# Farofeiro231/LiDAR_SLAM

Measured on AMD Instinct MI355X. Metric: scans/sec (RANSAC+UKF, 720-pt scans) at 1/2/4/8 MI355X + HBM GB/s vs peak, higher is better.
Workload: dtype f64; 1 GPU; C3: 4096 synthetic 720-pt scans per GPU, chunked 7x100+20; RANSAC (100 trials, 20 mm, mt19937 hypotheses) + landmark association + UKF predict/update (n=3, L=20); scans_per_gpu=4096, trials=100, landmarks=20, hyp=mt19937, parallelism=dp1 (scan shards, no collective)

## Files before the change

lidar_slam_amd/csrc/lslam_rng_pipe.h:

```cpp
#pragma once
#include "../../include/lidarslam.h"
#include "lslam_rng.h"

namespace lslam {

#ifndef RP_PRIO_TOP
#define RP_PRIO_TOP 3
#endif
__device__ __forceinline__ void set_prio_level(int lvl) {
    switch (lvl) {
        case 3: __builtin_amdgcn_s_setprio(3); break;
        case 2: __builtin_amdgcn_s_setprio(2); break;
        case 1: __builtin_amdgcn_s_setprio(1); break;
        default: __builtin_amdgcn_s_setprio(0); break;
    }
}

template <int LO, int HI>
__device__ __forceinline__ void mt_twist_group(const uint32_t *src, uint32_t *dst, uint32_t *pad, int lane) {
    uint32_t a[HI - LO], b[HI - LO], c[HI - LO];
#pragma unroll
    for (int k = LO; k < HI; k++) {
        const int i = 64 * k + lane;
        if (k < 9 || i < MT_N) {
            a[k - LO] = src[i];
            b[k - LO] = src[i + 1];
            const uint32_t *f = (i < MT_N - MT_M) ? src + i + MT_M : dst + i - (MT_N - MT_M);
            c[k - LO] = *f;
        }
    }
#pragma unroll
    for (int k = LO; k < HI; k++) {
        const int i = 64 * k + lane;
        if (k < 9 || i < MT_N) {
            const uint32_t v = mt_mix(a[k - LO], b[k - LO], c[k - LO]);
            dst[i] = v;
            if (k == 0 && pad) pad[lane] = v;
        }
    }
    wave_lds_sync();
}
__device__ __forceinline__ void mt_twist_oop(const uint32_t *src, uint32_t *dst, uint32_t *pad, int lane) {
    mt_twist_group<0, 3>(src, dst, pad, lane);
    mt_twist_group<3, 6>(src, dst, pad, lane);
    mt_twist_group<6, 9>(src, dst, pad, lane);
    mt_twist_group<9, 10>(src, dst, pad, lane);
}

constexpr uint32_t RT_KMAX = 127;
constexpr int RT_ROWS = 128;
constexpr int RT_ST = 7;
constexpr int RT_DWORDS = RT_ROWS * RT_ST;
__host__ __device__ inline uint32_t rt_word(uint32_t K, uint32_t v, uint32_t q) {
    uint32_t word = 0;
    for (uint32_t b = 0; b < 32; b++) {
        const uint32_t x = q * 32u + b;
        const uint32_t i = K - x % K;
        uint32_t m = i;
        m |= m >> 1; m |= m >> 2; m |= m >> 4; m |= m >> 8; m |= m >> 16;
        if ((v & m) > i) word |= 1u << b;
    }
    return word;
}

struct RngPipe;
__device__ __forceinline__ int rp_level(const RngPipe &rp, uint32_t done);

struct RngPipe {
    uint32_t *blk;
    int have;
    uint32_t *tbl;
    uint32_t tblK;
    uint32_t total_steps;
    uint32_t lvl_t1, lvl_t2;
    uint32_t done_steps;
    int prio;
#ifdef LSLAM_STAMPS
    uint64_t acc[8];
#endif
#ifdef LSLAM_WSTAMPS
    uint64_t wacc[8];
#endif
};

__device__ __forceinline__ void rp_set_schedule(RngPipe &rp) {
    rp.lvl_t1 = (rp.total_steps + 1u + 2u) / 3u;
    rp.lvl_t2 = (2u * (rp.total_steps + 1u) + 2u) / 3u;
}
__device__ __forceinline__ int rp_level(const RngPipe &rp, uint32_t done) {
    return RP_PRIO_TOP - (done >= rp.lvl_t1 ? 1 : 0) - (done >= rp.lvl_t2 ? 1 : 0);
}

__device__ __forceinline__ void rp_need_block(RngPipe &rp, int need, int lane) {
    if (rp.have < need) {
        mt_twist_oop(rp.blk + ((need - 1) & 1) * MT_N, rp.blk + (need & 1) * MT_N,
                     (need & 1) == 0 ? rp.blk + 2 * MT_N : nullptr, lane);
        rp.have = need;
    }
}

#if defined(LSLAM_STAMPS) && !defined(LSLAM_WSTAMPS)
#define RP_STAMP_DECL uint64_t _rp_prev = lslam_stamp();
#define RP_STAMP(k)                         \
    do {                                    \
        const uint64_t _t = lslam_stamp();  \
        rp.acc[k] += _t - _rp_prev;         \
        _rp_prev = _t;                      \
    } while (0)
#define RP_COUNT(k, n) (rp.acc[k] += (n))
#else
#define RP_STAMP_DECL
#define RP_STAMP(k) do {} while (0)
#define RP_COUNT(k, n) do {} while (0)
#endif

__device__ __forceinline__ uint32_t mbcnt_from(uint64_t m, uint32_t base) {
    return __builtin_amdgcn_mbcnt_hi((uint32_t)(m >> 32), __builtin_amdgcn_mbcnt_lo((uint32_t)m, base));
}

__device__ __forceinline__ uint32_t step_mask(uint32_t i) { return 0xffffffffu >> __clz((int)i); }

__device__ __forceinline__ uint32_t rt_temper_mask(uint32_t y, uint32_t mK) {
    y ^= (y >> 11);
    y = __builtin_amdgcn_bitop3_b32(y << 7, 0x9d2c5680u, y, 0x6a);
    y = __builtin_amdgcn_bitop3_b32(y << 15, 0xefc60000u, y, 0x6a);
    return (y ^ (y >> 18)) & mK;
}

__device__ __forceinline__ uint32_t fy_index(uint32_t d, uint32_t K) { return min(d, d + K) + 1u; }
__device__ __forceinline__ uint32_t fy_j(uint32_t w, uint32_t i) { return w & (0xffffffffu >> __clz((int)i)); }

__device__ __forceinline__ void store_accepted(uint8_t *J, uint32_t idx, uint32_t v, uint64_t R) {
    uint64_t saved;
    asm volatile(
        "s_andn1_saveexec_b64 %0, %1\n\t"
        "global_store_byte %2, %3, %4\n\t"
        "s_mov_b64 exec, %0"
        : "=&s"(saved)
        : "s"(R), "v"(idx), "v"(v), "s"(J)
        : "memory", "scc");
}
__device__ __forceinline__ void store_accepted(uint16_t *J, uint32_t idx, uint32_t v, uint64_t R) {
    uint64_t saved;
    asm volatile(
        "s_andn1_saveexec_b64 %0, %1\n\t"
        "global_store_short %2, %3, %4\n\t"
        "s_mov_b64 exec, %0"
        : "=&s"(saved)
        : "s"(R), "v"(idx * 2u), "v"(v), "s"(J)
        : "memory", "scc");
}

__device__ __forceinline__ uint32_t accepted_count(uint64_t R) {
    uint32_t n;
    asm("s_bcnt0_i32_b64 %0, %1" : "=s"(n) : "s"(R) : "scc");
    return n;
}

template <bool FAST, typename JT>
__device__ __forceinline__ void parse_chunk(RngPipe &rp, int &blkno, int &pos, JT *__restrict__ J, uint32_t N,
                                            uint32_t D, int lane) {
    const uint32_t K = N - 1;
    const uint32_t G = D * K;
    const float invK = 1.0f / (float)K;
    const uint32_t guess = ((uint32_t)lane * 46u) >> 6;
    uint32_t g = 0, sg = 0;
    int pre_pos = -1;
    uint32_t pre_raw = 0;
    RP_STAMP_DECL
    while (g < G) {
        RP_STAMP(3);
        if (pos >= MT_N) {
            blkno += 1;
            rp_need_block(rp, blkno, lane);
            asm volatile("" ::: "memory");
            pos -= MT_N;
            pre_pos = -1;
            const int lvl = rp_level(rp, rp.done_steps + g);
            if (lvl != rp.prio) {
                rp.prio = lvl;
                set_prio_level(lvl);
            }
            RP_STAMP(0);
        }
        const uint32_t *kb = rp.blk + (blkno & 1) * MT_N;
        const uint32_t rem = G - g;
        if (FAST) {
            rp_need_block(rp, blkno + 1, lane);
            asm volatile("" ::: "memory");
        }
        const int nrun = FAST ? min((MT_N - pos + 63) >> 6, (int)((rem - 1u) >> 6)) : 0;
        if (nrun > 0) {
            uint32_t raw = (pre_pos == pos) ? pre_raw : kb[pos + lane];
            uint32_t w = rt_temper_mask(raw, 0xffffffffu);
            for (int r = 0; r < nrun; r++) {
                const uint32_t nraw = kb[pos + 64 + lane];
                RP_STAMP(3);
                const uint32_t b1 = K - 1u - sg;
                const uint32_t base0 = b1 - (uint32_t)lane;
                uint32_t d = b1 - guess;
                uint32_t i = fy_index(d, K);
                uint32_t jv = fy_j(w, i);
                uint64_t R = ballot(jv > i), Rp;
                const uint32_t wn = rt_temper_mask(nraw, 0xffffffffu);
                int it = 1;
                do {
                    Rp = R;
                    d = mbcnt_from(Rp, base0);
                    i = fy_index(d, K);
                    jv = fy_j(w, i);
                    R = ballot(jv > i);
                    it++;
                } while (R != Rp);
                (void)it;
                RP_STAMP(2);
                RP_COUNT(5, 1);
                RP_COUNT(6, it);
                store_accepted(J, g + (b1 - d), jv, R);
                const uint32_t na = accepted_count(R);
                pos += 64;
                g += na;
                sg += na;
                if (sg >= K) sg -= K;
                raw = nraw;
                w = wn;
            }
            pre_pos = pos;
            pre_raw = raw;
            continue;
        }
        const uint32_t raw = (pre_pos == pos) ? pre_raw : kb[min(pos + lane, MT_N - 1)];
        pre_pos = -1;
        const uint32_t w = mt_temper(raw);
        RP_STAMP(3);
        const int nw = min(64, MT_N - pos);
        const uint64_t actm = ballot(lane < nw);
        uint32_t c = guess, jv = 0;
        uint64_t B = 0;
        for (int it = 0;; it++) {
            const uint32_t rr = sg + c;
            uint32_t r;
            if (FAST) {
                r = min(rr, rr - K);
            } else {
                uint32_t qq;
                divmod_small(rr, K, invK, qq, r);
            }
            const uint32_t i = K - r;
            jv = fy_j(w, i);
            const uint64_t Bn = actm & ballot(c < rem) & ballot(jv <= i);
            if (it > 0 && Bn == B) break;
            B = Bn;
            c = mbcnt(B);
        }
        RP_STAMP(2);
        RP_COUNT(5, 1);
        const uint32_t na = (uint32_t)popc64(B);
        if ((B >> lane) & 1ull) J[g + c] = (JT)jv;
        if (na >= rem && na > 0) {
            pos += fls64(B) + 1;
            pre_pos = -1;
        } else {
            pos += nw;
        }
        g += na;
        if (FAST) {
            sg += na;
            if (sg >= K) sg -= K;
        } else {
            uint32_t q, rs;
            divmod_small(sg + na, K, invK, q, rs);
            sg = rs;
        }
    }
    rp.done_steps += G;
}


__device__ __forceinline__ bool rt_rej(uint64_t M, uint32_t s) {
    uint32_t hi = (uint32_t)((M << s) >> 32);
    asm("" : "+v"(hi));
    return (int32_t)hi < 0;
}

template <bool KGE64>
__device__ __forceinline__ uint32_t rt_wrap(uint32_t x, uint32_t K) {
    x = min(x, x - K);
    if (!KGE64)
        while (x >= K) x -= K;
    return x;
}

typedef __attribute__((address_space(3))) const uint32_t lds_u32_t;
__device__ __forceinline__ uint64_t rt_window(const uint32_t *tbl, uint32_t v, uint32_t sg) {
    uint32_t q, base;
    asm("s_lshr_b32 %0, %1, 5" : "=s"(q) : "s"(sg) : "scc");
    asm("s_lshl2_add_u32 %0, %1, %2" : "=s"(base) : "s"(q), "s"((uint32_t)(uintptr_t)(lds_u32_t *)tbl) : "scc");
    lds_u32_t *row = (lds_u32_t *)(uintptr_t)(__umul24(v, RT_ST * 4u) + base);
    const uint32_t d0 = row[0], d1 = row[1], d2 = row[2];
    const uint32_t r = sg & 31u;
    const uint32_t lo = __builtin_amdgcn_alignbit(d1, d0, r);
    const uint32_t hi = __builtin_amdgcn_alignbit(d2, d1, r);
    return ((uint64_t)hi << 32) | lo;
}

template <bool KGE64, typename JT>
__device__ __forceinline__ void tbl_window(RngPipe &rp, const uint32_t *kb, int &pos, uint32_t &raw, uint32_t &gq,
                                           uint32_t &sg, JT *__restrict__ J, uint32_t K, uint32_t mK, uint32_t sbase,
                                           uint32_t s0, int lane) {
#ifdef LSLAM_WSTAMPS
    const bool wst = true;
    uint64_t _w = wst ? lslam_stamp() : 0;
#define WSTAMP(k)                                  \
    do {                                           \
        if (wst) {                                 \
            const uint64_t _t = lslam_stamp();     \
            rp.wacc[k] += _t - _w;                 \
            _w = _t;                               \
        }                                          \
    } while (0)
    if (wst) {
        WSTAMP(7);
        rp.wacc[5] += 1;
    }
#else
#define WSTAMP(k) do {} while (0)
#endif
    const uint32_t nraw = kb[pos + 64 + lane];
    const uint32_t v = rt_temper_mask(raw, mK);
    WSTAMP(0);
    const uint64_t M = rt_window(rp.tbl, v, sg);
#ifdef LSLAM_WSTAMPS
    if (wst) asm volatile("" ::"v"((uint32_t)M), "v"((uint32_t)(M >> 32)));
#endif
    WSTAMP(1);
#ifndef LSLAM_STAMPS
    uint32_t na, tS, tI;
    uint64_t tE;
#define TBL_EVAL_VCC                                \
    "v_mbcnt_lo_u32_b32 %[S], vcc_lo, %[sb]\n\t"  \
    "v_mbcnt_hi_u32_b32 %[S], vcc_hi, %[S]\n\t"   \
    "v_lshlrev_b64 v[28:29], %[S], %[M]\n\t"      \
    "s_nop 0\n\t"                                 \
    "v_cmp_gt_i32_e32 vcc, 0, v29\n\t"            \
    "s_nop 1\n\t"
#define TBL_TURNS                                                   \
    "v_lshlrev_b64 v[28:29], %[s0], %[M]\n\t"                     \
    "s_nop 0\n\t"                                                 \
    "v_cmp_gt_i32_e32 vcc, 0, v29\n\t"                            \
    "s_nop 1\n\t" TBL_EVAL_VCC TBL_EVAL_VCC                        \
    "TBLA_%=:\n\t"                                            \
    "v_mbcnt_lo_u32_b32 %[S], vcc_lo, %[sb]\n\t"                  \
    "v_mbcnt_hi_u32_b32 %[S], vcc_hi, %[S]\n\t"                   \
    "v_lshlrev_b64 v[28:29], %[S], %[M]\n\t"                      \
    "s_nop 0\n\t"                                                 \
    "v_cmp_gt_i32_e64 s[40:41], 0, v29\n\t"                       \
    "s_cmp_eq_u64 s[40:41], vcc\n\t"                              \
    "s_cbranch_scc1 TBLX_%=\n\t"                              \
    "v_mbcnt_lo_u32_b32 %[S], s40, %[sb]\n\t"                     \
    "v_mbcnt_hi_u32_b32 %[S], s41, %[S]\n\t"                      \
    "v_lshlrev_b64 v[28:29], %[S], %[M]\n\t"                      \
    "s_nop 0\n\t"                                                 \
    "v_cmp_gt_i32_e32 vcc, 0, v29\n\t"                            \
    "s_cmp_eq_u64 vcc, s[40:41]\n\t"                              \
    "s_cbranch_scc0 TBLA_%=\n"                                 \
    "TBLX_%=:\n\t"                                            \
    "v_sub_u32 %[I], %[gq], %[S]\n\t"
    if constexpr (sizeof(JT) == 1) {
        asm volatile(TBL_TURNS
                     "s_andn1_saveexec_b64 %[E], vcc\n\t"
                     "global_store_byte %[I], %[v], %[J]\n\t"
                     "s_mov_b64 exec, %[E]\n\t"
                     "s_bcnt0_i32_b64 %[na], vcc"
                     : [na] "=s"(na), [S] "=&v"(tS), [I] "=&v"(tI), [E] "=&s"(tE)
                     : [M] "v"(M), [s0] "v"(s0), [sb] "v"(sbase), [v] "v"(v), [gq] "s"(gq), [J] "s"(J)
                     : "vcc", "scc", "v28", "v29", "s40", "s41", "memory");
    } else {
        asm volatile(TBL_TURNS
                     "v_lshlrev_b32 %[I], 1, %[I]\n\t"
                     "s_andn1_saveexec_b64 %[E], vcc\n\t"
                     "global_store_short %[I], %[v], %[J]\n\t"
                     "s_mov_b64 exec, %[E]\n\t"
                     "s_bcnt0_i32_b64 %[na], vcc"
                     : [na] "=s"(na), [S] "=&v"(tS), [I] "=&v"(tI), [E] "=&s"(tE)
                     : [M] "v"(M), [s0] "v"(s0), [sb] "v"(sbase), [v] "v"(v), [gq] "s"(gq), [J] "s"(J)
                     : "vcc", "scc", "v28", "v29", "s40", "s41", "memory");
    }
#undef TBL_TURNS
#undef TBL_EVAL_VCC
#else
    uint64_t R = ballot(rt_rej(M, s0));
#pragma unroll
    for (int e = 0; e < 2; e++) R = ballot(rt_rej(M, mbcnt_from(R, sbase)));
#ifdef LSLAM_WSTAMPS
    if (wst) asm volatile("" ::"s"(R));
#endif
    WSTAMP(2);
    uint32_t s;
    RP_COUNT(6, 3);
    for (;;) {
        s = mbcnt_from(R, sbase);
        const uint64_t Rn = ballot(rt_rej(M, s));
        RP_COUNT(6, 1);
#ifdef LSLAM_WSTAMPS
        if (wst) rp.wacc[6] += 1;
#endif
        if (Rn == R) break;
        R = Rn;
    }
    RP_COUNT(5, 1);
    WSTAMP(3);
    store_accepted(J, gq - s, v, R);
    const uint32_t na = accepted_count(R);
#endif
    pos += 64;
    gq += na;
    sg = rt_wrap<KGE64>(sg + na, K);
    raw = nraw;
#ifdef LSLAM_WSTAMPS
    if (wst) asm volatile("" ::"s"(sg), "s"(gq));
#endif
    WSTAMP(4);
#undef WSTAMP
}

template <bool KGE64, typename JT>
__device__ __forceinline__ void parse_chunk_tbl(RngPipe &rp, int &blkno, int &pos, JT *__restrict__ J, uint32_t N,
                                                uint32_t D, int lane) {
    const uint32_t K = N - 1;
    const uint32_t G = D * K;
    const uint32_t mK = 0xffffffffu >> __clz((int)K);
    const uint32_t sbase = 63u - (uint32_t)lane;
    const uint32_t s0 = 63u - (((uint32_t)lane * 46u) >> 6);
    uint32_t g = 0, sg = 0;
    int pre_pos = -1;
    uint32_t pre_raw = 0;
    RP_STAMP_DECL
    while (g < G) {
        RP_STAMP(3);
        if (pos >= MT_N) {
            blkno += 1;
            rp_need_block(rp, blkno, lane);
            asm volatile("" ::: "memory");
            pos -= MT_N;
            pre_pos = -1;
            RP_STAMP(0);
        }
        rp_need_block(rp, blkno + 1, lane);
        asm volatile("" ::: "memory");
        const uint32_t *kb = rp.blk + (blkno & 1) * MT_N;
        const uint32_t rem = G - g;
        const int nrun = min((MT_N - pos + 63) >> 6, (int)((rem - 1u) >> 6));
        if (nrun > 0) {
            uint32_t raw = (pre_pos == pos) ? pre_raw : kb[pos + lane];
            uint32_t gq = g + 63u;
            const int pos_end = pos + 64 * nrun;
            if (nrun & 1) tbl_window<KGE64>(rp, kb, pos, raw, gq, sg, J, K, mK, sbase, s0, lane);
            while (pos != pos_end) {
                tbl_window<KGE64>(rp, kb, pos, raw, gq, sg, J, K, mK, sbase, s0, lane);
                tbl_window<KGE64>(rp, kb, pos, raw, gq, sg, J, K, mK, sbase, s0, lane);
            }
            g = gq - 63u;
            RP_STAMP(2);
            pre_pos = pos;
            pre_raw = raw;
            continue;
        }
        if (pos + 64 > MT_N) {
            rp_need_block(rp, blkno + 1, lane);
            asm volatile("" ::: "memory");
            pre_pos = -1;
        }
        const uint32_t raw = (pre_pos == pos) ? pre_raw : kb[pos + lane];
        pre_pos = -1;
        const uint32_t v = rt_temper_mask(raw, mK);
        const uint64_t M = rt_window(rp.tbl, v, sg);
        RP_STAMP(3);
        const int nw = 64;
        const uint64_t actm = ~0ull;
        const int thr = 63 - (int)min(rem, 64u);
        uint64_t A = actm & ballot(!rt_rej(M, s0) && (int)s0 > thr);
        uint32_t s;
        for (;;) {
            s = mbcnt_from(~A, sbase);
            const uint64_t An = actm & ballot(!rt_rej(M, s) && (int)s > thr);
            if (An == A) break;
            A = An;
        }
        RP_STAMP(2);
        RP_COUNT(5, 1);
        if ((A >> lane) & 1ull) J[(g + 63u) - s] = (JT)v;
        const uint32_t na = (uint32_t)popc64(A);
        if (na >= rem && na > 0) pos += fls64(A) + 1;
        else pos += nw;
        g += na;
        sg = rt_wrap<KGE64>(sg + na, K);
    }
    rp.done_steps += G;
}

template <typename JT>
__device__ __forceinline__ void resolve_draws_fwd(const JT *__restrict__ Js, uint32_t K, uint32_t d0, uint32_t D,
                                                  int32_t *__restrict__ draws, int lane) {
    const uint32_t d = d0 + (uint32_t)lane;
    const bool live = d < D;
    const JT *Jd = Js + (size_t)(live ? d : d0) * K;
    uint32_t c0 = 0, c1 = 1;
    for (uint32_t lo = 2; lo <= K;) {
        const uint32_t m = step_mask(lo);
        const uint32_t hi = min(K, m);
        uint32_t i = lo;
        for (; i + 8 <= hi + 1; i += 8) {
            uint32_t jj[8];
#pragma unroll
            for (int u = 0; u < 8; u++) jj[u] = Jd[K - i - u] & m;
#pragma unroll
            for (int u = 0; u < 8; u++) {
                c0 = (jj[u] == c0) ? i + u : c0;
                c1 = (jj[u] == c1) ? i + u : c1;
            }
        }
        for (; i <= hi; i++) {
            const uint32_t j = Jd[K - i] & m;
            c0 = (j == c0) ? i : c0;
            c1 = (j == c1) ? i : c1;
        }
        lo = hi + 1;
    }
    if (live) {
        const uint32_t j1 = Jd[K - 1] & 1u;
        draws[2 * d] = (int32_t)((j1 == 0u) ? c1 : c0);
        draws[2 * d + 1] = (int32_t)((j1 == 0u) ? c0 : c1);
    }
}

template <typename JT>
__device__ __forceinline__ void resolve_chunk(const JT *__restrict__ J, uint32_t K, uint32_t D, uint32_t stage_cap,
                                              unsigned char *stage, int32_t *__restrict__ draws, int lane) {
    const uint32_t bytes = D * K * (uint32_t)sizeof(JT);
    const uintptr_t gs = (uintptr_t)J;
    const uintptr_t a0 = gs & ~(uintptr_t)15;
    const uint32_t skew = (uint32_t)(gs - a0);
    const uint32_t n16 = (skew + bytes + 15u) >> 4;
    if (n16 * 16u <= stage_cap) {
        for (uint32_t e = (uint32_t)lane; e < n16; e += 64) ((uint4 *)stage)[e] = ((const uint4 *)a0)[e];
        __syncthreads();
        const JT *Js = (const JT *)(stage + skew);
        for (uint32_t d0 = 0; d0 < D; d0 += 64) resolve_draws_fwd(Js, K, d0, D, draws, lane);
    } else {
        for (uint32_t d0 = 0; d0 < D; d0 += 64) resolve_draws_fwd(J, K, d0, D, draws, lane);
    }
}

}
```

Baseline: 6.254 million scans/s.

## Replace modular wrap loop with magic-multiply reduction and unroll table window by four

For K below 64, the repeated-subtraction wrap of the shuffle cursor is replaced by a precomputed reciprocal multiply-high reduction. The table-window loop is unrolled four-way, with odd and two-step remainders handled first. An empty asm ties raw to gq to steer instruction scheduling, and the two alignbit operations are swapped. The aim is to cut serial scalar latency in the hot RNG parse loop, at the cost of code size and a reduction that relies on exactness of the magic constant for the small ranges used.

```diff
diff --git a/lidar_slam_amd/csrc/lslam_rng_pipe.h b/lidar_slam_amd/csrc/lslam_rng_pipe.h
--- a/lidar_slam_amd/csrc/lslam_rng_pipe.h
+++ b/lidar_slam_amd/csrc/lslam_rng_pipe.h
@@ -1,6 +1,7 @@
 #pragma once
 #include "../../include/lidarslam.h"
 #include "lslam_rng.h"
+#include "lslam_wrap.h"
 
 namespace lslam {
 
@@ -284,11 +285,9 @@
 }
 
 template <bool KGE64>
-__device__ __forceinline__ uint32_t rt_wrap(uint32_t x, uint32_t K) {
-    x = min(x, x - K);
-    if (!KGE64)
-        while (x >= K) x -= K;
-    return x;
+__device__ __forceinline__ uint32_t rt_wrap(uint32_t x, uint32_t K, uint32_t wm) {
+    if (KGE64) return min(x, x - K);
+    return rt_wrap_small(x, K, wm);
 }
 
 typedef __attribute__((address_space(3))) const uint32_t lds_u32_t;
@@ -299,15 +298,15 @@
     lds_u32_t *row = (lds_u32_t *)(uintptr_t)(__umul24(v, RT_ST * 4u) + base);
     const uint32_t d0 = row[0], d1 = row[1], d2 = row[2];
     const uint32_t r = sg & 31u;
+    const uint32_t hi = __builtin_amdgcn_alignbit(d2, d1, r);
     const uint32_t lo = __builtin_amdgcn_alignbit(d1, d0, r);
-    const uint32_t hi = __builtin_amdgcn_alignbit(d2, d1, r);
     return ((uint64_t)hi << 32) | lo;
 }
 
 template <bool KGE64, typename JT>
 __device__ __forceinline__ void tbl_window(RngPipe &rp, const uint32_t *kb, int &pos, uint32_t &raw, uint32_t &gq,
                                            uint32_t &sg, JT *__restrict__ J, uint32_t K, uint32_t mK, uint32_t sbase,
-                                           uint32_t s0, int lane) {
+                                           uint32_t s0, uint32_t wm, int lane) {
 #ifdef LSLAM_WSTAMPS
     const bool wst = true;
     uint64_t _w = wst ? lslam_stamp() : 0;
@@ -327,6 +326,7 @@
 #define WSTAMP(k) do {} while (0)
 #endif
     const uint32_t nraw = kb[pos + 64 + lane];
+    asm("" : "+v"(raw) : "s"(gq));
     const uint32_t v = rt_temper_mask(raw, mK);
     WSTAMP(0);
     const uint64_t M = rt_window(rp.tbl, v, sg);
@@ -415,7 +415,7 @@
 #endif
     pos += 64;
     gq += na;
-    sg = rt_wrap<KGE64>(sg + na, K);
+    sg = rt_wrap<KGE64>(sg + na, K, wm);
     raw = nraw;
 #ifdef LSLAM_WSTAMPS
     if (wst) asm volatile("" ::"s"(sg), "s"(gq));
@@ -432,6 +432,7 @@
     const uint32_t mK = 0xffffffffu >> __clz((int)K);
     const uint32_t sbase = 63u - (uint32_t)lane;
     const uint32_t s0 = 63u - (((uint32_t)lane * 46u) >> 6);
+    const uint32_t wm = KGE64 ? 0u : rt_wrap_magic(K);
     uint32_t g = 0, sg = 0;
     int pre_pos = -1;
     uint32_t pre_raw = 0;
@@ -455,11 +456,19 @@
             uint32_t raw = (pre_pos == pos) ? pre_raw : kb[pos + lane];
             uint32_t gq = g + 63u;
             const int pos_end = pos + 64 * nrun;
-            if (nrun & 1) tbl_window<KGE64>(rp, kb, pos, raw, gq, sg, J, K, mK, sbase, s0, lane);
+#define TBL_WIN() tbl_window<KGE64>(rp, kb, pos, raw, gq, sg, J, K, mK, sbase, s0, wm, lane)
+            if (nrun & 1) TBL_WIN();
+            if (nrun & 2) {
+                TBL_WIN();
+                TBL_WIN();
+            }
             while (pos != pos_end) {
-                tbl_window<KGE64>(rp, kb, pos, raw, gq, sg, J, K, mK, sbase, s0, lane);
-                tbl_window<KGE64>(rp, kb, pos, raw, gq, sg, J, K, mK, sbase, s0, lane);
+                TBL_WIN();
+                TBL_WIN();
+                TBL_WIN();
+                TBL_WIN();
             }
+#undef TBL_WIN
             g = gq - 63u;
             RP_STAMP(2);
             pre_pos = pos;
@@ -494,7 +503,7 @@
         if (na >= rem && na > 0) pos += fls64(A) + 1;
         else pos += nw;
         g += na;
-        sg = rt_wrap<KGE64>(sg + na, K);
+        sg = rt_wrap<KGE64>(sg + na, K, wm);
     }
     rp.done_steps += G;
 }
diff --git a/lidar_slam_amd/csrc/lslam_wrap.h b/lidar_slam_amd/csrc/lslam_wrap.h
--- /dev/null
+++ b/lidar_slam_amd/csrc/lslam_wrap.h
@@ -0,0 +1,15 @@
+#pragma once
+#include <stdint.h>
+
+#if defined(__HIPCC__)
+#define LSLAM_WRAP_FN __host__ __device__ __forceinline__
+#else
+#define LSLAM_WRAP_FN static inline
+#endif
+
+LSLAM_WRAP_FN uint32_t rt_wrap_magic(uint32_t K) { return 0xffffffffu / K + 1u; }
+
+LSLAM_WRAP_FN uint32_t rt_wrap_small(uint32_t x, uint32_t K, uint32_t m) {
+    const uint32_t q = (uint32_t)(((uint64_t)x * m) >> 32);
+    return x - q * K;
+}
```

New measurement: 6.275 million scans/s, median of 6. No clear change (+0.3%).
